# xacond00/mitsuba3-amvpt

Hardware: AMD Instinct MI355X
Metric: Msamples/sec (whole node), 8-view 1024² 64spp; per-pixel RMSE vs llvm_rgb (higher is better)
Workload: dtype f32; 1 GPU; M: cbox_grid.xml, 8-view 1024x1024 per view (quilt 4096x2048), 64 spp (4 passes x 16), G=8, sa_mis, adaptive 0, max_depth 8, rr_depth 5, seed 0; partition=equal lane counts, film_bytes_per_gpu=134217728

## Files before the change

include/amvpt.h:

```cpp
#ifndef AMVPT_H
#define AMVPT_H

#include <stddef.h>
#include <stdint.h>

#ifdef __cplusplus
extern "C" {
#endif

#define AMVPT_ABI_VERSION 10

typedef enum amvpt_status {
    AMVPT_OK = 0,
    AMVPT_ERR_INVALID = 1,
    AMVPT_ERR_HIP = 2,
    AMVPT_ERR_OOM = 3,
    AMVPT_ERR_UNSUPPORTED = 4,
    AMVPT_ERR_NO_DEVICE = 5
} amvpt_status;


enum {
    AMVPT_SHAPE_RECTANGLE = 0,
    AMVPT_SHAPE_MESH = 1,
    AMVPT_SHAPE_SPHERE = 2
};

typedef struct amvpt_shape_desc {
    uint32_t type;
    int32_t bsdf;
    int32_t emitter;
    uint32_t flip_normals;
    float to_world[16];
    float to_object[16];
    uint32_t vertex_count;
    uint32_t face_count;
    const float *positions;
    const float *normals;
    const float *texcoords;
    const uint32_t *faces;
    float center[3];
    float radius;
} amvpt_shape_desc;

enum {
    AMVPT_BSDF_DIFFUSE = 0,
    AMVPT_BSDF_ROUGHCONDUCTOR = 1,
    AMVPT_BSDF_TWOSIDED = 2
};
enum { AMVPT_MICROFACET_BECKMANN = 0, AMVPT_MICROFACET_GGX = 1 };

typedef struct amvpt_bsdf_desc {
    uint32_t type;
    int32_t nested[2];
    float reflectance[3];
    uint32_t distribution;
    uint32_t sample_visible;
    float alpha_u, alpha_v;
    float eta[3], k[3];
    uint32_t has_specular_reflectance;
    float specular_reflectance[3];
} amvpt_bsdf_desc;

// ... 121 lines not shown
amvpt_status amvpt_scene_destroy(amvpt_scene *scene);
amvpt_status amvpt_scene_stats(const amvpt_scene *scene, uint32_t *n_nodes, uint32_t *n_prims);
amvpt_status amvpt_scene_desc_boxes(const amvpt_scene_desc *d, uint32_t *n_boxes);

uint32_t amvpt_film_channels(const amvpt_params *params);

amvpt_status amvpt_render(amvpt_scene *scene, const amvpt_view_desc *views,
                          const amvpt_params *params, uint64_t lane_begin,
                          uint64_t lane_end, float *film_device, void *stream,
                          amvpt_counters *counters);

amvpt_status amvpt_render_records(amvpt_scene *scene, const amvpt_view_desc *views,
                                  const amvpt_params *params, uint32_t pass,
                                  uint64_t lane_begin, uint64_t lane_end, float *film_device,
                                  float *records_device, void *stream);

amvpt_status amvpt_plan(const amvpt_params *params, uint32_t *spp, uint32_t *spp_per_pass,
                        uint32_t *n_passes, uint64_t *lanes_per_pass);

amvpt_status amvpt_develop(const float *film_device, float *out_device, uint32_t width,
                           uint32_t height, uint32_t film_alpha, void *stream);

amvpt_status amvpt_set_chunk_lanes(uint64_t chunk_lanes);
amvpt_status amvpt_set_traversal(uint32_t mode);
amvpt_status amvpt_set_bvh_build(uint32_t max_leaf_prims, float traversal_cost);

typedef int (*amvpt_exchange_fn)(void *ctx, uint64_t local_count, uint64_t *prefix, uint64_t *total);
amvpt_status amvpt_set_adaptive_exchange(amvpt_exchange_fn fn, void *ctx);


typedef struct amvpt_lane_set {
    uint64_t lane_begin, lane_end;
    uint32_t rect_x0, rect_y0, rect_width, rect_height;
} amvpt_lane_set;

typedef struct amvpt_film_window {
    float *film;
    uint32_t x0, y0, width, height;
    uint32_t *overflow;
    uint64_t overflow_capacity;
} amvpt_film_window;

typedef int (*amvpt_run_exchange_fn)(void *ctx, uint32_t n_runs, const uint64_t *run_lane_begin,
                                     const uint64_t *run_count, uint64_t *run_prefix, uint64_t *total);

enum {
    AMVPT_OPT_GENERIC_KERNELS = 1u,
    AMVPT_OPT_WAVEFRONT_SUFFIX = 2u,
    AMVPT_OPT_SPLIT_NEE = 4u,
    AMVPT_OPT_ONE_STREAM = 8u,
    AMVPT_OPT_NO_BINNING = 32u,
    AMVPT_OPT_NO_BOX_SCREEN = 64u,
    AMVPT_OPT_THREADED_BVH = 128u,
    AMVPT_OPT_DETERMINISTIC = 16u
};
typedef struct amvpt_render_opts {
    uint64_t chunk_lanes;
    uint32_t traversal;
    uint32_t flags;
    amvpt_run_exchange_fn exchange;
    void *exchange_ctx;
    float *records;
    uint32_t record_pass;
    uint32_t budget_mib;
} amvpt_render_opts;

amvpt_status amvpt_render_ex(amvpt_scene *scene, const amvpt_view_desc *views, const amvpt_params *params,
                             const amvpt_lane_set *lanes, const amvpt_film_window *film, void *stream,
                             const amvpt_render_opts *opts, amvpt_counters *counters);

amvpt_status amvpt_film_accumulate(float *quilt, uint32_t quilt_width, uint32_t quilt_height, uint32_t channels,
                                   const float *window, uint32_t x0, uint32_t y0, uint32_t width, uint32_t height,
                                   const uint32_t *overflow_entries, uint64_t n_entries, void *stream);

amvpt_status amvpt_release_device_memory(int device);

amvpt_status amvpt_scene_bvh2(const amvpt_scene *scene, uint32_t *n_nodes2, uint32_t *depth);

#ifdef __cplusplus
}
#endif

#endif
```

mitsuba3-amvpt_amd/amvpt/__init__.py:

```python
import ctypes
import os

import numpy as np

_HERE = os.path.dirname(os.path.abspath(__file__))
LIB_DIR = os.environ.get("AMVPT_LIB_DIR") or os.path.join(os.path.dirname(_HERE), "lib")
HIP_LIB_PATH = os.path.join(LIB_DIR, "libamvpt_hip.so")
HOST_LIB_PATH = os.path.join(LIB_DIR, "libamvpt_host.so")

u32, i32, u64, f32, f64 = ctypes.c_uint32, ctypes.c_int32, ctypes.c_uint64, ctypes.c_float, ctypes.c_double


class ShapeDesc(ctypes.Structure):
    _fields_ = [("type", u32), ("bsdf", i32), ("emitter", i32), ("flip_normals", u32),
                ("to_world", f32 * 16), ("to_object", f32 * 16),
                ("vertex_count", u32), ("face_count", u32),
                ("positions", ctypes.POINTER(f32)), ("normals", ctypes.POINTER(f32)),
                ("texcoords", ctypes.POINTER(f32)), ("faces", ctypes.POINTER(u32)),
                ("center", f32 * 3), ("radius", f32)]


class BsdfDesc(ctypes.Structure):
    _fields_ = [("type", u32), ("nested", i32 * 2), ("reflectance", f32 * 3), ("distribution", u32),
                ("sample_visible", u32), ("alpha_u", f32), ("alpha_v", f32), ("eta", f32 * 3),
# ... 20 lines not shown


class Params(ctypes.Structure):
    _fields_ = [(n, u32) for n in (
        "integrator", "max_depth", "rr_depth", "hide_emitters", "sa_reuse", "sa_mis", "fast_mis",
        "debug", "adaptive", "spp_pass_lim", "reuse_count", "spp", "seed", "base_seed", "n_views",
        "multisensor", "grid_x", "grid_y", "reverse_x", "reverse_y", "film_width", "film_height",
        "film_alpha", "rfilter")] + [("rfilter_stddev", f32), ("batch", u32), ("crop_offset_x", u32),
                                      ("crop_offset_y", u32), ("full_width", u32), ("full_height", u32)]


class Counters(ctypes.Structure):
    _fields_ = [("lanes", u64), ("passes", u64), ("vertices", u64), ("reuse_lanes", u64),
                ("visibility_rays", u64), ("view_splats", u64), ("adaptive_lanes", u64),
                ("kernel_ms_primary", f64), ("kernel_ms_bounce", f64), ("kernel_ms_splat", f64),
                ("total_ms", f64), ("splat_fallback", u64),
                ("shadow_rays", u64), ("kernel_ms", f64 * 12), ("kernel_launches", u64 * 12),
                ("record_bytes", u64), ("nonfinite_samples", u64), ("negative_samples", u64),
                ("pushed_paths", u64), ("film_overflow", u64), ("film_range_drops", u64),
                ("chunk_lanes", u64), ("buffer_sets", u64), ("arena_bytes", u64),
                ("primary_record_bytes", u64), ("splat_record_bytes", u64)]

    def as_dict(self):
        d = {k: getattr(self, k) for k, _ in self._fields_}
        for k in ("kernel_ms", "kernel_launches"):
            d[k] = {name: d[k][i] for i, name in enumerate(KERNELS)}
        return d


class LaneSet(ctypes.Structure):
    _fields_ = [("lane_begin", u64), ("lane_end", u64), ("rect_x0", u32), ("rect_y0", u32),
                ("rect_width", u32), ("rect_height", u32)]


class FilmWindow(ctypes.Structure):
    _fields_ = [("film", ctypes.c_void_p), ("x0", u32), ("y0", u32), ("width", u32), ("height", u32),
                ("overflow", ctypes.c_void_p), ("overflow_capacity", u64)]


RunExchangeFn = ctypes.CFUNCTYPE(ctypes.c_int, ctypes.c_void_p, u32, ctypes.POINTER(u64), ctypes.POINTER(u64),
                                 ctypes.POINTER(u64), ctypes.POINTER(u64))


class RenderOpts(ctypes.Structure):
    _fields_ = [("chunk_lanes", u64), ("traversal", u32), ("flags", u32), ("exchange", RunExchangeFn),
                ("exchange_ctx", ctypes.c_void_p), ("records", ctypes.c_void_p), ("record_pass", u32),
                ("budget_mib", u32)]


OPT_GENERIC_KERNELS, OPT_WAVEFRONT_SUFFIX, OPT_SPLIT_NEE, OPT_ONE_STREAM, OPT_DETERMINISTIC = 1, 2, 4, 8, 16
OPT_NO_BINNING = 32
OPT_NO_BOX_SCREEN = 64
OPT_THREADED_BVH = 128


def wrap_run_exchange(fn):
    def cb(_ctx, n, begins, counts, prefix, total):
        try:
            pre, tot = fn([int(begins[i]) for i in range(n)], [int(counts[i]) for i in range(n)])
            for i in range(n):
                prefix[i] = int(pre[i])
            total[0] = int(tot)
            return 0
        except Exception:
            return 1
    return RunExchangeFn(cb)


KERNELS = ("k_prim_hit", "k_prim_req", "k_vis", "k_mv_primary", "k_raygen", "k_extend", "k_bounce", "k_shadow",
           "k_splat", "k_suffix", "k_select", "k_bin")


INTEGRATOR_MVPATH, INTEGRATOR_PATH = 0, 1
EMITTER_AREA, EMITTER_CONSTANT = 0, 1
_hip = None
_host = None


def hip_lib():
    global _hip
    if _hip is None:
        if not os.path.exists(HIP_LIB_PATH):
            raise RuntimeError("libamvpt_hip.so missing: run `make -C mitsuba3-amvpt_amd` "
                               "(__graft_entry__.build()); the product path has no fallback")
        L = ctypes.CDLL(HIP_LIB_PATH, mode=ctypes.RTLD_GLOBAL)
        L.amvpt_last_error.restype = ctypes.c_char_p
        L.amvpt_abi_version.restype = u32
        L.amvpt_film_channels.restype = u32
        for fn in ("amvpt_device_count", "amvpt_set_device", "amvpt_scene_create", "amvpt_scene_destroy",
                   "amvpt_scene_stats", "amvpt_render", "amvpt_render_records", "amvpt_plan",
                   "amvpt_develop", "amvpt_set_chunk_lanes", "amvpt_set_traversal",
                   "amvpt_set_adaptive_exchange", "amvpt_set_bvh_build", "amvpt_render_ex", "amvpt_scene_desc_boxes",
                   "amvpt_release_device_memory"):
            if hasattr(L, fn):
                getattr(L, fn).restype = ctypes.c_int
        L.amvpt_render.argtypes = [ctypes.c_void_p, ctypes.c_void_p, ctypes.POINTER(Params), u64, u64,
                                   ctypes.c_void_p, ctypes.c_void_p, ctypes.POINTER(Counters)]
        if hasattr(L, "amvpt_render_ex"):
            L.amvpt_render_ex.argtypes = [ctypes.c_void_p, ctypes.c_void_p, ctypes.POINTER(Params),
                                          ctypes.POINTER(LaneSet), ctypes.POINTER(FilmWindow), ctypes.c_void_p,
                                          ctypes.POINTER(RenderOpts), ctypes.POINTER(Counters)]
        L.amvpt_render_records.argtypes = [ctypes.c_void_p, ctypes.c_void_p, ctypes.POINTER(Params), u32, u64,
                                           u64, ctypes.c_void_p, ctypes.c_void_p, ctypes.c_void_p]
        L.amvpt_scene_create.argtypes = [ctypes.POINTER(SceneDesc), ctypes.POINTER(ctypes.c_void_p)]
        L.amvpt_scene_destroy.argtypes = [ctypes.c_void_p]
        L.amvpt_scene_stats.argtypes = [ctypes.c_void_p, ctypes.POINTER(u32), ctypes.POINTER(u32)]
# ... 326 lines not shown
```

mitsuba3-amvpt_amd/csrc/amvpt_render.hip:

```cpp
#include <hip/hip_runtime.h>
#include <rocprofiler-sdk-roctx/roctx.h>

#include <algorithm>
#include <chrono>
#include <cmath>
#include <cstdlib>
#include <cstring>
#include <map>
#include <memory>
#include <mutex>
#include <type_traits>

#include "internal.h"
#include "dbsdf.h"

#if defined(AMVPT_SHADOW_TU) || defined(AMVPT_GROUP_TU)
#define AMVPT_TU_LOCAL static
#else
#define AMVPT_TU_LOCAL
#endif

namespace amvpt {

#if !defined(AMVPT_SHADOW_TU) && !defined(AMVPT_GROUP_TU)
// ... 18 lines not shown
        Hit best{kInf, 0.f, 0.f, -1};
        uint32_t best_orig = 0xffffffffu;
        outer_closest(sc, r, best, best_orig);
        return trace_closest2<walk_sph<kWalk>()>(sc, r, best, best_orig);
    }
    return trace_closest<kWalk == WALK_UNI, AMVPT_WALK_WW, walk_sph<kWalk>()>(sc, r);
}
template <int kWalk> AD bool walk_any(const SceneRef &sc, const Ray &r) {
    if (kWalk == WALK_BRUTE || kWalk == WALK_BRUTE_NS) return brute_any<kWalk == WALK_BRUTE>(sc, r);
    if (kWalk != WALK_UNI && sc.stk) return trace_any2<walk_sph<kWalk>()>(sc, r, outer_any(sc, r, false));
    return trace_any<kWalk == WALK_UNI, AMVPT_WALK_WW, walk_sph<kWalk>()>(sc, r);
}

struct KParams {
    uint32_t W, H, C;
    uint32_t bvh2, stk_off_ext, stk_off_any;
    uint32_t spp_pp, log_spp, pow2;
    uint32_t max_depth, rr_depth;
    uint32_t sa_mis, fast_mis, debug, n_adapt;
    uint32_t G;
    uint32_t multisensor, batch, n_views, gx, gy, rev_x, rev_y, sres_x, sres_y;
    uint32_t needs_ap;
    uint32_t box, coalesce_single, path_box_pos, is_mvpath;
    uint32_t seed_value;
    uint32_t trav_mode;
    uint32_t sph;
    uint32_t win_rs;
    uint32_t adapt_seed;
    uint32_t pass_seed;
    uint64_t range_begin;
    uint32_t rect, rect_x0, rect_y0, run_len;
    uint32_t fx0, fy0, fw, fh;
    uint32_t *overflow;
    uint64_t ov_cap;
    float inv_w, inv_h;
    uint32_t off_x, off_y;
    float adj_ox, adj_oy, nc_ox, nc_oy;
    float adapt_w;
    FilterCoeffs filt;
    uint64_t chunk_begin;
    uint32_t chunk_n;
    uint32_t record;
    uint32_t row_splat;
    uint32_t tile_w;
    double rcp_tpr, rcp_run_len, rcp_n_adapt;
    uint32_t adapt_pass;
    uint32_t valid_ray0;
    uint32_t vs_stride;
    unsigned long long *film_fx;
    float *film_base;
    unsigned long long *fx_drops;
    unsigned long long *rng_in, *rng_out;
    uint32_t box_screen;
    float bin_lo[3], bin_scale[3];
};

AD Pcg pass_rng(const KParams &P, uint32_t lane, uint64_t v) {
    uint32_t v0, v1;
    tea4(P.seed_value, lane, v0, v1);
    Pcg rng;
    if (P.rng_in) {
        rng.state = P.rng_in[v];
        rng.inc = (((uint64_t) v1) << 1) | 1u;
    } else {
        rng.seed(v0, v1);
    }
    return rng;
}

constexpr int kQPlanes = 5;
struct Bufs {
    float4 *q_in[kQPlanes];
    float4 *q_out[kQPlanes];
    uint32_t *cnt_in, *cnt_out;
    uint32_t qcap;
    float4 *lane_out;
    float4 *lrec[4];
    float4 *vrec;
    float *film;
    float *records;
    unsigned long long *stats;
    uint8_t *amask;
    const uint32_t *asel;
    const uint32_t *run_delta;
    float4 *hit;
    float4 *nee[2];
    float2 *nee_gb;
    uint32_t *cnt_nee;
    float4 *vreq[3];
    unsigned long long *occ;
    uint4 *vreq_w[8];
    uint4 *lmask_w[24];
    float *vstate;
    float4 *sray[2];
    float2 *sgb;
    uint16_t *key_out, *key_in, *key_nee;
};


constexpr int kPrimBlock = 128;
enum { F_PDF, F_JP, F_PDFM, F_WX, F_WY, F_WZ, VS_FIELDS };
constexpr int kVsFieldsDiff = 2;

__host__ __device__ inline bool scene_uniform(uint32_t n_nodes, uint32_t mode) {
    return mode == 1u || (mode == 0u && n_nodes <= kUniformNodeLimit);
}
// ... 2213 lines not shown

#ifndef AMVPT_BOUNCE_TAB
#define AMVPT_BOUNCE_TAB 1
#endif
#ifndef AMVPT_PRIM_TAB
#define AMVPT_PRIM_TAB 1
#endif
#ifndef AMVPT_PRIM_SLOT_ORDER
#define AMVPT_PRIM_SLOT_ORDER 1
#endif
#ifndef AMVPT_DEFER_SAMPLE
#define AMVPT_DEFER_SAMPLE 1
#endif
#ifndef AMVPT_PAIR_REGS
#define AMVPT_PAIR_REGS 1
#endif
#ifndef AMVPT_PDF_REGS
#define AMVPT_PDF_REGS 1
#endif
#ifndef AMVPT_DIFF_REGS
#define AMVPT_DIFF_REGS 0
#endif
template <int G, bool kDiff> __host__ __device__ constexpr bool diff_regs() {
    return AMVPT_DIFF_REGS && AMVPT_PAIR_REGS && kDiff && G >= 2 && G <= 8;
}
template <int G, bool kDiff> __host__ __device__ constexpr bool pdf_in_regs() {
    return (AMVPT_PAIR_REGS && AMVPT_PDF_REGS && !kDiff && G >= 2 && G <= 8) || diff_regs<G, kDiff>();
}
template <int G, bool kDiff> __host__ __device__ constexpr int vs_fields() {
    return kDiff ? (diff_regs<G, kDiff>() ? 0 : kVsFieldsDiff) : VS_FIELDS - (pdf_in_regs<G, kDiff>() ? 1 : 0);
}
#ifndef AMVPT_FUSED_TWO_STREAMS
#define AMVPT_FUSED_TWO_STREAMS 0
#endif
#ifndef AMVPT_CHUNK_STREAMS
#define AMVPT_CHUNK_STREAMS 4
#endif
#ifndef AMVPT_TILE_SLOTS
#define AMVPT_TILE_SLOTS 1
#endif
#ifndef AMVPT_PDF_ROW
#define AMVPT_PDF_ROW 1
#endif
#ifndef AMVPT_COH_UNI
#define AMVPT_COH_UNI 1
#endif
#ifndef AMVPT_WAVE_DIFF
#define AMVPT_WAVE_DIFF 1
#endif
#ifndef AMVPT_PRIM_WAVES
#define AMVPT_PRIM_WAVES 1
#endif
template <int G> constexpr int prim_block() { return G > 0 ? kPrimBlock : 64; }
template <int G, bool kTab, bool kDiff, bool kGenRec>
AD void mv_primary_lane(const KParams &P, const DScene &S, const SceneRef &sc, const DView *V, const Bufs &B,
                        float *const vs, const uint32_t vs_stride, const uint32_t slot, const uint32_t i, const bool ok) {
    const int Gn = group_size<G>(P);
    constexpr bool kPdfRegs = pdf_in_regs<G, kDiff>();
    constexpr bool kJpRegs = diff_regs<G, kDiff>();
#define VSF(f, k) vs[(((f) - (kPdfRegs ? 1 : 0)) * Gn + (k)) * vs_stride]
    PathState ps;
    bool push = false;
    unsigned long long st_reuse = 0, st_vis = 0;
    if (ok) {
        const float4 hitv = B.hit[i];
        VMask<G> occm = 0;
#pragma unroll
        for (int k = 0; k < Gn; ++k) mset(occm, k, occluded_n(B, (uint32_t) Gn, i, k));
        const uint32_t n = P.chunk_n;
        const PrimRay pr = primary_raygen(P, V, i);
        Pcg rng = pr.rng;
        const uint32_t v1 = pr.v1, p_idx = pr.p_idx;
        const float apx = pr.apx, apy = pr.apy;
        const Ray pray = pr.ray;
        float *const vw = kGenRec ? vrec_compact(B, Gn, n) : reinterpret_cast<float *>(B.vrec);
        float4 *const vR = B.vrec, *const vB = B.vrec + (size_t) Gn * n;
        auto view_of = [&](int k) -> uint32_t { return group_view_n((uint32_t) Gn, p_idx, k); };
        auto put_view = [&](int k, float w, C3 res, C3 bv, uint32_t vf) {
            const size_t o = (size_t) k * n + slot;
            if (kDiff) {
                vw[o] = w;
            } else {
                vR[o] = make_float4(res.r, res.g, res.b, w);
                vB[o] = make_float4(bv.r, bv.g, bv.b, bitsf(vf));
            }
        };
        VMask<G> vmask = 0, imask = 0;
        float w0 = 1.f;
        C3 R0 = c3(0.f);
        C3 Dp = c3(0.f);
        C3 Bv = c3(0.f);
        f3 hp = mk(0.f, 0.f, 0.f);
        bool records_done = false, reuse_l = false, direct_l = false;
        uint32_t nf_bits = 0;
        VMask<G> smask = 0;

        bool valid_ray = P.valid_ray0 != 0 && P.max_depth != 0, adapt_mask = false;
        float pdfW = 1.f;
        bool should_mis = P.sa_mis != 0;
        if (P.max_depth != 0) {
            SI si = compute_si(sc, pray, hit_of(hitv));
            bool p_hit = si.valid();
            hp = si.p;
            int32_t em = si_emitter(sc, si);
            bool direct_em = em >= 0;
            C3 emitted = c3(0.f);
            if (direct_em) emitted = emitter_eval(sc, em, si, true);
            int32_t b = p_hit ? S.shapes[si.shape].bsdf : -1;
            bool bsdf_smooth = (bsdf_flags(S.bsdfs, b) & BF_Smooth) != 0;
            bool active_em = p_hit && bsdf_smooth;
            float e1 = rng.next_1d(), e2 = rng.next_1d();
            DSamp ds;
            C3 em_w;
            if (sample_emitter_direction(sc, si, e1, e2, active_em, ds, em_w) && mget(occm, 0))
                occlude_emitter_sample(ds, em_w);
            active_em = active_em && ds.pdf != 0.f;
            direct_l = active_em;
            f3 wo = si.sh.to_local(ds.d);
            float rand_1 = rng.next_1d();
            float r2a = rng.next_1d(), r2b = rng.next_1d();
            (void) rand_1;
            C3 bsdf_val;
            float direct_pdf;
            bsdf_eval_pdf<kDiff>(S.bsdfs, b, CTX_ALL, si.wi, wo, true, bsdf_val, direct_pdf);
            BSample bsmp;
            C3 bsdf_weight;
            bsdf_sample<kDiff>(S.bsdfs, b, CTX_ALL, si.wi, r2a, r2b, true, bsmp, bsdf_weight);
            bool flag_delta = (bsmp.type & BF_Delta) != 0, flag_null = (bsmp.type & BF_Null) != 0;
            bool flag_diff = (bsmp.type & BF_Diffuse) != 0;
            bool delta = flag_delta || flag_null, p_not_delta = !delta && p_hit;
            bool reuse = !direct_em && p_not_delta && bsdf_smooth;
            reuse_l = reuse;
            st_reuse += reuse ? 1 : 0;
            bool p_face = si.wi.z > 0.f;
            if (should_mis) {
                BD bd;
                bd.bsdf = b;
                bd.alpha = bsdf_roughness<kDiff>(S.bsdfs, b, si.wi);
                bd.sqr_a = fmsub(bd.alpha, bd.alpha, 1.f);
                bd.rsqrt_a = rsqrt_(bd.alpha);
                bd.diffuse = flag_diff;
                bd.reuse = reuse;
                Surf p0 = camera_sample_surface(V[view_of(0)], si, p_hit, apx, apy);
                const float pdf0 = p0.pdf, Jp0 = p0.Jp, iJp0 = p_hit ? rcp(p0.Jp) : 0.f;
                if (!kPdfRegs) VSF(F_PDF, 0) = pdf0;
                float rJp[kJpRegs ? G : 1];
                if constexpr (kJpRegs) {
                    rJp[0] = Jp0;
#pragma unroll
                    for (int j = 1; j < G; ++j) rJp[j] = 0.f;
                } else {
                    VSF(F_JP, 0) = Jp0;
                }
                mset(vmask, 0, p_hit);
                mset(imask, 0, p_hit);
                const f3 wo_r0 = reflect_l(si.wi);
                VMask<G> wpos = p_face ? 1u : 0u;
                if (!kDiff) {
                    VSF(F_WX, 0) = si.wi.x; VSF(F_WY, 0) = si.wi.y; VSF(F_WZ, 0) = si.wi.z;
                    VSF(F_PDFM, 0) = bd.diffuse ? 1.f : (P.fast_mis ? sqr(normalize(si.wi + wo_r0).z)
                                                                   : bsdf_pdf(S.bsdfs, b, CTX_GLOSSY, si.wi, wo_r0, p_hit));
                }
                auto wi_of = [&](int k) -> f3 {
                    if (kDiff) return k == 0 ? si.wi : mk(0.f, 0.f, mget(wpos, k) ? 1.f : -1.f);
                    return mk(VSF(F_WX, k), VSF(F_WY, k), VSF(F_WZ, k));
                };
                auto mat_pdf = [&](f3 wik, float pdfM, bool active) -> float {
                    if (bd.diffuse) return 1.f;
                    return P.fast_mis ? tv_pdf_fast(wo_r0, wik, pdfM, bd, active)
                                      : tv_pdf(S.bsdfs, wo_r0, wik, pdfM, bd, active);
                };
                float rPdf[kPdfRegs ? G : 1];
                if constexpr (kPdfRegs) {
#pragma unroll
                    for (int j = 0; j < G; ++j) rPdf[j] = 0.f;
                }
                float n_direct = 1.f, n_indir = 2.f;
                int rep_k = 0;
                (void) rep_k;
#pragma unroll 1
                for (int k = 1; k < Gn; ++k) {
                    Surf r = camera_sample_surface(V[view_of(k)], si, bd.reuse, apx, apy);
                    bool valid = r.valid && (r.face == p_face) && r.Jp > 0.f;
                    if (valid) {
                        ++st_vis;
                        valid = !mget(occm, k);
                    }
                    f3 wik = si.sh.to_local(r.d);
                    float pdf_Mat = 1.f;
                    if (!kDiff) {
                        VSF(F_WX, k) = wik.x; VSF(F_WY, k) = wik.y; VSF(F_WZ, k) = wik.z;
                        f3 wor = reflect_l(wik);
                        float pdfM = P.fast_mis ? sqr(normalize(wik + wor).z)
                                                : bsdf_pdf(S.bsdfs, b, CTX_GLOSSY, wik, wor, valid);
                        VSF(F_PDFM, k) = pdfM;
                        pdf_Mat = mat_pdf(wik, pdfM, valid);
                    } else {
                        mset(wpos, k, wik.z > 0.f);
                    }
                    float J = r.Jp * iJp0;
                    float pdf_J = J > 1.f ? rcp(J) : J;
                    float pdf_Sel = pdf_Mat * pdf_J;
                    valid = valid && (rng.next_1d() < pdf_Sel);
                    if constexpr (kJpRegs) {
#pragma unroll
                        for (int j = 1; j < G; ++j) rJp[j] = j == k ? r.Jp : rJp[j];
                    } else {
                        VSF(F_JP, k) = r.Jp;
                    }
                    if constexpr (kPdfRegs) {
                        const float pk = valid ? r.pdf : 0.f;
#pragma unroll
                        for (int j = 1; j < G; ++j) rPdf[j] = j == k ? pk : rPdf[j];
                    } else {
                        VSF(F_PDF, k) = valid ? r.pdf : 0.f;
                    }
                    bool indirect = valid, direct = valid;
                    bool replace = n_indir * rng.next_1d() < 1.f;
                    C3 bvk;
                    float bpk;
                    BSample bsk;
                    C3 bwk;
                    bsdf_eval_pdf<kDiff>(S.bsdfs, b, CTX_ALL, wik, wo, valid, bvk, bpk);
                    direct = direct && bpk > 0.f;
                    direct_pdf += direct ? bpk : 0.f;
                    n_direct += (float) direct;
                    if (!kDiff) {
#if AMVPT_DEFER_SAMPLE
                        indirect = indirect && bsdf_sample_type(S.bsdfs, b, CTX_ALL, wik, valid) == bsmp.type;
                        if (indirect && replace) rep_k = k;
#else
                        bsdf_sample(S.bsdfs, b, CTX_ALL, wik, r2a, r2b, valid, bsk, bwk);
                        indirect = indirect && bsk.type == bsmp.type;
                        if (indirect && replace) bsmp.wo = bsk.wo;
#endif
                    }
                    (void) replace;
                    n_indir += (float) indirect;
                    mset(vmask, k, valid);
// ... 122 lines not shown
                            if (j == k) continue;
                            float pdf_J = vmin(sqr(VSF(F_JP, j) * iJpk), 1.f);
                            acc = fmadd(VSF(F_PDF, j), pdf_J, acc);
                        }
                        acc = cond ? acc : 0.f;
                    }
                    pdfSum += acc;
                    const float wk = pdf_lk / pdfSum;
                    bool valid = mget(imask, k);
                    C3 res = c3(0.f), bv = c3(0.f);
                    float bp;
                    if (kDiff) {
                        bp = (valid && mget(wpos, k)) ? bp_d : 0.f;
                    } else {
                        res = csel(k == 0, emitted, c3(0.f));
                        if (active_em && vk) {
                            C3 bvk = bsdf_val;
                            if (k > 0) {
                                float bpk;
                                bsdf_eval_pdf<kDiff>(S.bsdfs, b, CTX_ALL, wik, wo, true, bvk, bpk);
                            }
                            res = cfma(bvk, emis_mis, res);
                        }
                        if (k == 0) R0 = res;
                        bsdf_eval_pdf<kDiff>(S.bsdfs, b, CTX_ALL, wik, bsmp.wo, valid, bv, bp);
                        if (k == 0) {
                            bv = csel(p_not_delta, bv, bsdf_weight);
                            bp = p_not_delta ? bp : bsmp.pdf;
                            valid = valid && (bp > 0.f || delta);
                        }
                    }
                    bool pvalid = bp > 0.f;
                    valid = valid && ((k == 0 && !kDiff) ? (pvalid || delta) : pvalid);
                    bp = valid ? bp : 0.f;
                    bv = csel(valid, bv, c3(0.f));
                    pdf += bp;
                    n_ind += (float) valid;
                    if (!valid) mclr(imask, k);
                    if (k == 0) w0 = wk;
                    else put_view(k, wk, res, bv, (vk ? VF_VALID : 0u) | (valid ? VF_INDIRECT : 0u));
                    if (k == 0 && !kDiff) Bv = bv;
                }
                bsmp.pdf = p_not_delta ? pdf / n_ind : bsmp.pdf;
                adapt_mask = p_hit && !flag_null && (n_ind <= 1.f);
                records_done = true;
            } else {
                mset(vmask, 0, p_hit);
#pragma unroll 1
                for (int k = 1; k < Gn; ++k) {
                    Surf r = camera_sample_surface(V[view_of(k)], si, reuse, apx, apy);
                    bool valid = r.valid && (r.face == p_face) && r.Jp > 0.f;
                    if (valid) {
                        ++st_vis;
                        valid = !mget(occm, k);
                    }
                    mset(vmask, k, valid);
                }
                float mis_em = ds.delta ? 1.f : mis_weight(ds.pdf, direct_pdf);
                R0 = emitted;
                if (active_em) R0 = cfma(bsdf_val, em_w * mis_em, R0);
            }
            Ray pd_ray = spawn_ray(si.p, si.n, si.sh.to_world(bsmp.wo));
            C3 thr = csel(should_mis, c3(1.f), bsdf_weight);
            valid_ray = valid_ray || (p_hit && !flag_null);
            bool pd_active = p_hit;
            if (!should_mis) pd_active = pd_active && (cmax(thr) != 0.f);
            if (P.max_depth <= 1) pd_active = false;
            pdfW = p_not_delta ? rcp(bsmp.pdf) : 1.f;
            if (pd_active) {
                ps.ray = pd_ray;
                ps.thr = thr;
                ps.res = c3(0.f);
                ps.eta_zero = bsmp.eta == 0.f;
                ps.prev_pdf = bsmp.pdf;
                ps.depth = p_hit ? 1u : 0u;
                ps.prev_delta = flag_delta;
                ps.valid_ray = false;
                ps.prev_p = si.p;
                ps.idx = slot;
                ps.rng_state = rng.state;
                ps.rng_seq = v1;
                push = true;
            }
            if (!p_hit) w0 = 1.f;
            mset(vmask, 0, true);
        }
        if (!push) B.lane_out[slot] = make_float4(0.f, 0.f, 0.f, 0.f);
        if (P.max_depth == 0) {
            vmask = 0u;
            imask = 0u;
            w0 = 0.f;
        }
        const uint32_t lflags = (valid_ray ? LF_VALIDRAY : 0u) | (adapt_mask ? LF_ADAPT : 0u) |
                                (should_mis ? LF_MIS : 0u) | (reuse_l ? LF_REUSE : 0u) | (direct_l ? LF_DIRECT : 0u) |
                                (nf_bits << 8) | mlow16(smask) | (kGenRec ? LF_DIFFW : 0u);
        B.lrec[0][slot] = make_float4(R0.r, R0.g, R0.b, pdfW);
        B.lrec[1][slot] = make_float4(Dp.r, Dp.g, Dp.b, bitsf(lflags));
        B.lrec[2][slot] = make_float4(Bv.r, Bv.g, Bv.b, bitsf(mlow16(vmask) >> 16 | mlow16(imask)));
        if constexpr (G <= 0) {
            constexpr int NP = mask_planes<G>();
            mstore(B.lmask_w, slot, vmask);
            mstore(B.lmask_w + NP, slot, imask);
            mstore(B.lmask_w + 2 * NP, slot, smask);
        }
        B.lrec[3][slot] = make_float4(hp.x, hp.y, hp.z, 0.f);
        put_view(0, w0, R0, Bv, (mget(vmask, 0) ? VF_VALID : 0u) | (mget(imask, 0) ? VF_INDIRECT : 0u));
        if (!records_done) {
#pragma unroll 1
            for (int k = 1; k < Gn; ++k)
                put_view(k, P.max_depth != 0 ? 1.f : 0.f, c3(0.f), c3(0.f), (mget(vmask, k)) ? VF_VALID : 0u);
        }
    }
    const uint32_t qslot = push_slot(push, B.cnt_out, B.qcap);
    if (push) store_state(B.q_out, qslot, ps);
    if (B.stats) {
        stat_add(B.stats, 1, st_reuse);
        stat_add(B.stats, 2, st_vis);
        stat_add(B.stats, 0, (ok && P.max_depth != 0) ? 1ull : 0ull);
        stat_add(B.stats, 8, push ? 1ull : 0ull);
        stat_add(B.stats, 10, ok ? (unsigned long long) ((kDiff ? 4 : 32) * Gn) : 0ull);
    }
}
#undef VSF

AD bool wave_diffuse(const KParams &P, const DScene &S, const SceneRef &sc, const Bufs &B, uint32_t i, bool ok) {
    bool dl = true;
    if (ok && P.max_depth != 0) {
        const int32_t prim = (int32_t) fbits(B.hit[i].w);
        if (prim >= 0) {
            const int32_t b = S.shapes[sc.prims[prim].shape].bsdf;
            dl = b < 0 || S.bsdfs[b].type == BSDF_DIFFUSE;
        }
    }
    return !wave_any(!dl);
}
template <int G, bool kTab, bool kDiff, bool kDW = false>
__global__ void __launch_bounds__(prim_block<G>(), AMVPT_PRIM_WAVES) k_mv_primary(KParams P, const DScene *Sp, const DView *V, Bufs B) {
    constexpr int kPB = prim_block<G>();
    extern __shared__ __attribute__((aligned(16))) char lds[];
    DScene S = *Sp;
    const uint32_t vs_off = kTab ? S.tab_bytes + views_lds_bytes(P.n_views) : 0u;
    SceneRef sc = stage_scene<kTab, false>(S, lds, P.trav_mode, &V, P.n_views);
    const bool vs_glob = G <= 0 && B.vstate != nullptr;
    const uint32_t vs_stride = vs_glob ? P.vs_stride : (uint32_t) kPB;
    float *const vs = vs_glob ? B.vstate + (blockIdx.x * blockDim.x + threadIdx.x)
                              : reinterpret_cast<float *>(lds + vs_off) + threadIdx.x;
#if AMVPT_PRIM_SLOT_ORDER
    const uint32_t slot = blockIdx.x * blockDim.x + threadIdx.x;
    bool ok = slot < P.chunk_n;
    const uint32_t i = ok ? slot_lane(P, slot) : 0u;
#else
    const uint32_t i = blockIdx.x * blockDim.x + threadIdx.x;
    bool ok = i < P.chunk_n;
    const uint32_t slot = ok ? lane_slot(P, i) : 0u;
#endif
    if constexpr (kDiff) {
        mv_primary_lane<G, kTab, true, false>(P, S, sc, V, B, vs, vs_stride, slot, i, ok);
    } else if (kDW) {
        if (wave_diffuse(P, S, sc, B, i, ok)) mv_primary_lane<G, kTab, true, true>(P, S, sc, V, B, vs, vs_stride, slot, i, ok);
    } else {
        if (!(AMVPT_WAVE_DIFF && wave_diffuse(P, S, sc, B, i, ok)))
            mv_primary_lane<G, kTab, false, false>(P, S, sc, V, B, vs, vs_stride, slot, i, ok);
    }
}



#ifndef AMVPT_SPLAT_SKIP
#define AMVPT_SPLAT_SKIP 1
#endif
#ifndef AMVPT_SPLAT_BVW
#define AMVPT_SPLAT_BVW 1
#endif
#ifndef AMVPT_SPLAT_WAVES
#define AMVPT_SPLAT_WAVES 5
#endif
template <int G, int C, bool kDiff, bool kRow, bool kWin = true, bool kRec = true>
__global__ void __launch_bounds__(kSplatBlock, AMVPT_SPLAT_WAVES) k_splat_multi(KParams P, const DView *V, Bufs B) {
    const bool rec_ = kRec && P.record != 0, dbg_ = kRec && P.debug != 0;
    __shared__ typename std::conditional<kRow, WaveLds<C>, SplatLds<C>>::type L;
    if (kRow) wave_lds_init(reinterpret_cast<WaveLds<C> &>(L));
    else splat_lds_init(reinterpret_cast<SplatLds<C> &>(L));
    auto put = [&](float x, float y, const float *vals, bool valid, bool coalesce, int buf, uint32_t *fb) {
        if constexpr (kRow) {
            wave_put<C, kWin>(P, B.film, L, x, y, vals, valid, coalesce, fb);
        } else {
            if (P.film_fx) direct_put<C, kWin>(P, B.film, x, y, vals, valid, coalesce);
            else block_put<C>(P, B.film, L, buf, x, y, vals, valid, coalesce, fb);
        }
    };
    const uint32_t slot = blockIdx.x * kSplatBlock + threadIdx.x;
    const bool ok = slot < P.chunk_n;
    const uint32_t i = ok ? slot_lane(P, slot) : 0u;
    const uint32_t n = P.chunk_n;
    float4 l0 = make_float4(0.f, 0.f, 0.f, 0.f), l1 = l0, l2 = l0, l3 = l0, lo = l0;
    if (ok) { l0 = B.lrec[0][slot]; l1 = B.lrec[1][slot]; l2 = B.lrec[2][slot]; l3 = B.lrec[3][slot]; lo = B.lane_out[slot]; }
    const int Gn = group_size<G>(P);
    const uint32_t lflags = fbits(l1.w);
    VMask<G> vmask = 0u, imask = 0u, smask = 0u;
    if constexpr (G <= 0) {
        constexpr int NP = mask_planes<G>(), NW = mask_words<G>();
        if (ok) { vmask = mload<NW>(B.lmask_w, slot); imask = mload<NW>(B.lmask_w + NP, slot); smask = mload<NW>(B.lmask_w + 2 * NP, slot); }
    } else {
        vmask = fbits(l2.w) & 0xffffu; imask = fbits(l2.w) >> 16; smask = lflags >> 16;
    }
    const float qnan = __builtin_nanf("");
    const float pdfW = l0.w;
    const C3 R0 = C3{l0.x, l0.y, l0.z}, Dp = C3{l1.x, l1.y, l1.z}, Bv = C3{l2.x, l2.y, l2.z};
    const f3 hp = mk(l3.x, l3.y, l3.z);
    if (ok && B.amask) B.amask[P.chunk_begin + i] = (lflags & LF_ADAPT) ? 1u : 0u;
// ... 87 lines not shown
        if (dbg_) {
            if (k > 0) break;
            pack_vals(P, c3(adapt_mask ? 1.f : 0.f), alpha, 1.f, vals);
            put(x, y, vals, ok, true, 0, nullptr);
            continue;
        }
        pack_vals(P, v, alpha, weight, vals);
        check_sample(P, vals, valid, nonfinite, negative);
        put(x, y, vals, valid, k == 0, k & 1, &fallback);
        splats += valid ? 1 : 0;
        if (ok && rec_) {
            float *rr = B.records + ((size_t) i * Gn + k) * 8;
            rr[0] = x; rr[1] = y; rr[2] = v.r; rr[3] = v.g; rr[4] = v.b; rr[5] = alpha; rr[6] = weight;
            rr[7] = valid ? 1.f : 0.f;
        }
    }
    if (B.stats) {
        stat_add(B.stats, 3, splats); stat_add(B.stats, 4, fallback);
        stat_add(B.stats, 6, nonfinite); stat_add(B.stats, 7, negative);
        const uint32_t vb = !ok ? 0u : kd ? 4u * views_read
                                          : 16u * ((rec_ ? views_read : mpopc(vmask)) + (mis ? mpopc(imask) : 0u));
        stat_add(B.stats, 11, vb);
    }
}

AMVPT_TU_LOCAL __global__ void k_develop(const float *film, float *out, uint32_t npx, uint32_t alpha) {
    uint32_t p = blockIdx.x * blockDim.x + threadIdx.x;
    if (p >= npx) return;
    uint32_t C = alpha ? 5u : 4u, T = alpha ? 4u : 3u;
    const float *src = film + (size_t) p * C;
    float w = src[C - 1];
    float d = w == 0.f ? 1.f : w;
    for (uint32_t c = 0; c < T; ++c) out[(size_t) p * T + c] = src[c] / d;
}

void launch_shadow(int walk, bool bin, dim3 grid, size_t lds, hipStream_t st, const KParams &P, const DScene *dS, const Bufs &B)
#ifdef AMVPT_SHADOW_TU
{
    if (bin && walk == WALK_LANE_TRI) hipLaunchKernelGGL(HIP_KERNEL_NAME(k_shadow<WALK_LANE_TRI, true>), grid, dim3(256), lds, st, P, dS, B);
    else if (bin && walk == WALK_LANE_NS) hipLaunchKernelGGL(HIP_KERNEL_NAME(k_shadow<WALK_LANE_NS, true>), grid, dim3(256), lds, st, P, dS, B);
    else if (bin && walk == WALK_LANE) hipLaunchKernelGGL(HIP_KERNEL_NAME(k_shadow<WALK_LANE, true>), grid, dim3(256), lds, st, P, dS, B);
    else if (walk == WALK_BRUTE_NS) hipLaunchKernelGGL(HIP_KERNEL_NAME(k_shadow<WALK_BRUTE_NS>), grid, dim3(256), lds, st, P, dS, B);
    else if (walk == WALK_BRUTE) hipLaunchKernelGGL(HIP_KERNEL_NAME(k_shadow<WALK_BRUTE>), grid, dim3(256), lds, st, P, dS, B);
    else if (walk == WALK_UNI) hipLaunchKernelGGL(HIP_KERNEL_NAME(k_shadow<WALK_UNI>), grid, dim3(256), lds, st, P, dS, B);
    else if (walk == WALK_LANE_TRI) hipLaunchKernelGGL(HIP_KERNEL_NAME(k_shadow<WALK_LANE_TRI>), grid, dim3(256), lds, st, P, dS, B);
    else if (walk == WALK_LANE_NS) hipLaunchKernelGGL(HIP_KERNEL_NAME(k_shadow<WALK_LANE_NS>), grid, dim3(256), lds, st, P, dS, B);
    else hipLaunchKernelGGL(HIP_KERNEL_NAME(k_shadow<WALK_LANE>), grid, dim3(256), lds, st, P, dS, B);
}
#else
;
#endif

struct AbKnobs {
    bool fuse_prim = true, row_splat = true, brute = true, fuse_nee = true, fuse_suffix = true;
    uint32_t win_rs = AMVPT_WIN_RS, fused_blocks = AMVPT_FUSED_BLOCKS;
};
inline const AbKnobs &ab_knobs() {
    static const AbKnobs k = [] {
        AbKnobs r;
#ifdef AMVPT_AB_KNOBS
        auto off = [](const char *n) { const char *e = std::getenv(n); return e && e[0] == '0'; };
        r.fuse_prim = !off("AMVPT_FUSE_PRIM");
        r.row_splat = !off("AMVPT_ROW_SPLAT");
        r.brute = !off("AMVPT_BRUTE");
        r.fuse_nee = !off("AMVPT_FUSE_NEE");
        r.fuse_suffix = !off("AMVPT_FUSE_SUFFIX");
        if (const char *e = std::getenv("AMVPT_WIN_RS")) r.win_rs = (uint32_t) std::strtoul(e, nullptr, 0) % 32u;
        if (const char *e = std::getenv("AMVPT_FUSED_BLOCKS"))
            r.fused_blocks = std::max<uint32_t>(1, std::min<uint32_t>(64, (uint32_t) std::strtoul(e, nullptr, 0)));
#endif
        return r;
    }();
    return k;
}

#ifndef AMVPT_FLUSH_MARKS
#define AMVPT_FLUSH_MARKS 1
#endif
struct KTimer {
    static constexpr size_t kPairs = 128;
    bool on = false;
    hipError_t err = hipSuccess;
    hipEvent_t ev[2 * kPairs] = {};
    int kid[kPairs] = {};
    size_t n = 0;
    double ms[AMVPT_K_COUNT] = {};
    uint64_t launches[AMVPT_K_COUNT] = {};
    void init(bool enable) {
        on = enable;
        if (!on) return;
        for (auto &e : ev)
            if (err == hipSuccess) err = hipEventCreate(&e);
    }
    void flush() {
        if (!on || n == 0 || err != hipSuccess) return;
        for (size_t i = 0; i < n && err == hipSuccess; ++i) {
            err = hipEventSynchronize(ev[2 * i + 1]);
            if (err != hipSuccess) break;
            float t = 0.f;
            err = hipEventElapsedTime(&t, ev[2 * i], ev[2 * i + 1]);
            ms[kid[i]] += t;
            launches[kid[i]] += 1;
        }
        n = 0;
    }
    void begin(int k, hipStream_t st) {
        if (!on || err != hipSuccess) return;
        if (n == kPairs) flush();
        kid[n] = k;
        err = hipEventRecord(ev[2 * n], st);
    }
    void end(hipStream_t st) {
        if (!on || err != hipSuccess) return;
        err = hipEventRecord(ev[2 * n + 1], st);
        ++n;
    }
    hipEvent_t mark_ev = nullptr;
    void mark(hipStream_t st) {
        if (on || !AMVPT_FLUSH_MARKS) return;
        if (!mark_ev && hipEventCreate(&mark_ev) != hipSuccess) return;
        (void) hipEventRecord(mark_ev, st);
    }
    ~KTimer() {
        for (auto &e : ev)
            if (e) (void) hipEventDestroy(e);
        if (mark_ev) (void) hipEventDestroy(mark_ev);
    }
};

void launch_prim_hit(bool uni, dim3 grid, size_t lds_bvh, hipStream_t st, const KParams &P, const DScene *S,
                     const DView *V, const Bufs &B)
#if !defined(AMVPT_SHADOW_TU) && !defined(AMVPT_GROUP_TU)
{
    if (uni) hipLaunchKernelGGL(HIP_KERNEL_NAME(k_prim_hit<true>), grid, dim3(256), lds_bvh, st, P, S, V, B);
    else hipLaunchKernelGGL(HIP_KERNEL_NAME(k_prim_hit<false>), grid, dim3(256), lds_bvh, st, P, S, V, B);
}
#else
;
#endif
#ifdef AMVPT_GROUP_TU
template <int G> inline int group_size_host(const KParams &P) { return G > 0 ? G : (int) P.G; }
template <int G>
void launch_primary(uint32_t cn, size_t lds_tab, size_t lds_bvh, hipStream_t st, const KParams &P,
                           const DScene *S, const DView *V, const Bufs &B, bool tab, bool uni, bool diff, KTimer &T) {
    constexpr int kPB = prim_block<G>(), kVW = vis_waves<G>();
    const dim3 g256((cn + 255) / 256), g64((cn + 63) / 64), gp((cn + kPB - 1) / kPB);
    const size_t lds_view = B.vstate ? 0u : (size_t) (diff ? vs_fields<G, true>() : vs_fields<G, false>()) * group_size_host<G>(P) * kPB * sizeof(float);
    if (uni && ab_knobs().fuse_prim) {
        T.begin(AMVPT_K_PRIM_HIT, st);
        if (tab && diff && P.sph == 0) hipLaunchKernelGGL(HIP_KERNEL_NAME(k_prim_hit_req<G, true, true, 0>), g256, dim3(256), lds_tab, st, P, S, V, B);
        else if (tab && P.sph == 0) hipLaunchKernelGGL(HIP_KERNEL_NAME(k_prim_hit_req<G, true, false, 0>), g256, dim3(256), lds_tab, st, P, S, V, B);
        else if (tab && diff && P.sph == 2) hipLaunchKernelGGL(HIP_KERNEL_NAME(k_prim_hit_req<G, true, true, 2>), g256, dim3(256), lds_tab, st, P, S, V, B);
        else if (tab && P.sph == 2) hipLaunchKernelGGL(HIP_KERNEL_NAME(k_prim_hit_req<G, true, false, 2>), g256, dim3(256), lds_tab, st, P, S, V, B);
        else if (tab && diff) hipLaunchKernelGGL(HIP_KERNEL_NAME(k_prim_hit_req<G, true, true>), g256, dim3(256), lds_tab, st, P, S, V, B);
        else if (tab) hipLaunchKernelGGL(HIP_KERNEL_NAME(k_prim_hit_req<G, true, false>), g256, dim3(256), lds_tab, st, P, S, V, B);
        else if (diff) hipLaunchKernelGGL(HIP_KERNEL_NAME(k_prim_hit_req<G, false, true>), g256, dim3(256), lds_tab, st, P, S, V, B);
        else hipLaunchKernelGGL(HIP_KERNEL_NAME(k_prim_hit_req<G, false, false>), g256, dim3(256), lds_tab, st, P, S, V, B);
        T.end(st);
    } else {
        T.begin(AMVPT_K_PRIM_HIT, st);
        launch_prim_hit(uni, g256, lds_bvh, st, P, S, V, B);
        T.end(st);
        T.begin(AMVPT_K_PRIM_REQ, st);
        if (tab && diff) hipLaunchKernelGGL(HIP_KERNEL_NAME(k_prim_req<G, true, true>), g256, dim3(256), lds_tab, st, P, S, V, B);
        else if (tab) hipLaunchKernelGGL(HIP_KERNEL_NAME(k_prim_req<G, true, false>), g256, dim3(256), lds_tab, st, P, S, V, B);
        else if (diff) hipLaunchKernelGGL(HIP_KERNEL_NAME(k_prim_req<G, false, true>), g256, dim3(256), lds_tab, st, P, S, V, B);
        else hipLaunchKernelGGL(HIP_KERNEL_NAME(k_prim_req<G, false, false>), g256, dim3(256), lds_tab, st, P, S, V, B);
        T.end(st);
    }
    T.begin(AMVPT_K_VIS, st);
    constexpr bool kVisPairs = vis_pairs<G, true>();
    const dim3 gvis = kVisPairs ? dim3((cn + 64 * AMVPT_VIS_RAYS - 1) / (64 * AMVPT_VIS_RAYS)) : g64;
    if (uni && P.sph == 0) hipLaunchKernelGGL(HIP_KERNEL_NAME(k_vis<G, true, 0>), gvis, dim3(64 * kVW), lds_bvh, st, P, S, V, B);
    else if (uni && P.sph == 2) hipLaunchKernelGGL(HIP_KERNEL_NAME(k_vis<G, true, 2>), gvis, dim3(64 * kVW), lds_bvh, st, P, S, V, B);
    else if (uni) hipLaunchKernelGGL(HIP_KERNEL_NAME(k_vis<G, true>), gvis, dim3(64 * kVW), lds_bvh, st, P, S, V, B);
    else hipLaunchKernelGGL(HIP_KERNEL_NAME(k_vis<G, false>), g64, dim3(64 * kVW), lds_bvh, st, P, S, V, B);
    T.end(st);
    T.begin(AMVPT_K_MV_PRIMARY, st);
    if (tab && diff) hipLaunchKernelGGL(HIP_KERNEL_NAME(k_mv_primary<G, true, true>), gp, dim3(kPB), lds_tab + lds_view, st, P, S, V, B);
    else if (diff) hipLaunchKernelGGL(HIP_KERNEL_NAME(k_mv_primary<G, false, true>), gp, dim3(kPB), lds_tab + lds_view, st, P, S, V, B);
    else {
        if (AMVPT_WAVE_DIFF) {
            const size_t lds_dw = B.vstate ? 0u : (size_t) vs_fields<G, true>() * group_size_host<G>(P) * kPB * sizeof(float);
            if (tab) hipLaunchKernelGGL(HIP_KERNEL_NAME(k_mv_primary<G, true, false, true>), gp, dim3(kPB), lds_tab + lds_dw, st, P, S, V, B);
            else hipLaunchKernelGGL(HIP_KERNEL_NAME(k_mv_primary<G, false, false, true>), gp, dim3(kPB), lds_tab + lds_dw, st, P, S, V, B);
        }
        if (tab) hipLaunchKernelGGL(HIP_KERNEL_NAME(k_mv_primary<G, true, false>), gp, dim3(kPB), lds_tab + lds_view, st, P, S, V, B);
        else hipLaunchKernelGGL(HIP_KERNEL_NAME(k_mv_primary<G, false, false>), gp, dim3(kPB), lds_tab + lds_view, st, P, S, V, B);
    }
    T.end(st);
}
template <int G>
void launch_splat(dim3 grid, hipStream_t st, const KParams &P, const DView *V, const Bufs &B, bool diff) {
    const bool row = AMVPT_WAVE_WIN && P.row_splat && P.C == 4 && !P.film_fx;
    const bool whole = P.fx0 == 0u && P.fy0 == 0u && P.fw == P.W && P.fh == P.H;
    if (P.C == 5 && diff) hipLaunchKernelGGL(HIP_KERNEL_NAME(k_splat_multi<G, 5, true, false>), grid, dim3(kSplatBlock), 0, st, P, V, B);
    else if (P.C == 5) hipLaunchKernelGGL(HIP_KERNEL_NAME(k_splat_multi<G, 5, false, false>), grid, dim3(kSplatBlock), 0, st, P, V, B);
    else if (diff && row && whole && !P.record && !P.debug) hipLaunchKernelGGL(HIP_KERNEL_NAME(k_splat_multi<G, 4, true, true, false, false>), grid, dim3(kSplatBlock), 0, st, P, V, B);
    else if (row && whole && !P.record && !P.debug) hipLaunchKernelGGL(HIP_KERNEL_NAME(k_splat_multi<G, 4, false, true, false, false>), grid, dim3(kSplatBlock), 0, st, P, V, B);
    else if (diff && row && whole) hipLaunchKernelGGL(HIP_KERNEL_NAME(k_splat_multi<G, 4, true, true, false>), grid, dim3(kSplatBlock), 0, st, P, V, B);
// ... 359 lines not shown
    const bool partial = rect || lane_begin != 0 || lane_end != L;
    const amvpt_run_exchange_fn exchange = opts.exchange;
    void *const exchange_ctx = opts.exchange_ctx;
    if (do_fill && partial && !exchange) {
        set_error("amvpt_render: adaptive > 0 over a lane range needs amvpt_set_adaptive_exchange "
                  "(or the whole frame: lane_begin = 0, lane_end = all lanes)");
        return AMVPT_ERR_UNSUPPORTED;
    }
    if (span == 0) {
        if (do_fill && partial)
            for (uint32_t pass = 0; pass < n_passes; ++pass) {
                uint64_t total = 0;
                if (exchange(exchange_ctx, 0, nullptr, nullptr, nullptr, &total) != 0) {
                    set_error("amvpt_render: adaptive count exchange failed");
                    return AMVPT_ERR_INVALID;
                }
            }
        if (counters) *counters = amvpt_counters{};
        return AMVPT_OK;
    }

    KParams P{};
    P.W = Pp.film_width; P.H = Pp.film_height; P.C = Pp.film_alpha ? 5 : 4;
    P.spp_pp = spp_pp;
    uint32_t log_spp = 0;
    while ((1u << log_spp) < spp_pp) ++log_spp;
    P.log_spp = log_spp;
    P.pow2 = (1u << log_spp) == spp_pp;
    P.max_depth = Pp.max_depth; P.rr_depth = Pp.rr_depth;
    P.sa_mis = Pp.sa_mis; P.fast_mis = Pp.fast_mis; P.debug = Pp.debug; P.n_adapt = n_adapt;
    P.G = G;
    P.multisensor = Pp.multisensor; P.batch = Pp.batch; P.n_views = Pp.n_views;
    P.needs_ap = 0;
    for (uint32_t v = 0; v < (Pp.multisensor && Pp.batch ? Pp.n_views : 1u); ++v)
        P.needs_ap |= views[v].type == AMVPT_CAMERA_THINLENS ? 1u : 0u;
    P.gx = Pp.grid_x ? Pp.grid_x : 1; P.gy = Pp.grid_y ? Pp.grid_y : 1;
    P.rev_x = Pp.reverse_x; P.rev_y = Pp.reverse_y;
    const uint32_t fullW = Pp.full_width ? Pp.full_width : P.W, fullH = Pp.full_height ? Pp.full_height : P.H;
    P.sres_x = fullW / P.gx; P.sres_y = fullH / P.gy;
    P.box = Pp.rfilter == AMVPT_RFILTER_BOX;
    P.coalesce_single = spp_pp >= 4;
    P.path_box_pos = (!is_mv && P.box) ? 1 : 0;
    P.is_mvpath = is_mv;
    P.inv_w = 1.f / (float) P.W;
    P.inv_h = 1.f / (float) P.H;
    P.off_x = Pp.crop_offset_x; P.off_y = Pp.crop_offset_y;
    P.adj_ox = -(float) P.off_x * P.inv_w;
    P.adj_oy = -(float) P.off_y * P.inv_h;
    P.nc_ox = (float) (-(int) P.off_x) - .5f;
    P.nc_oy = (float) (-(int) P.off_y) - .5f;
    P.adapt_w = 1.f / (float) (n_adapt + 1);
    P.trav_mode = trav;
    P.box_screen = (opts.flags & AMVPT_OPT_NO_BOX_SCREEN) ? 0u : 1u;
    for (int a = 0; a < 3; ++a) {
        const float ext = scene->root_hi[a] - scene->root_lo[a];
        P.bin_lo[a] = scene->root_lo[a];
        P.bin_scale[a] = ext > 0.f ? (float) (1u << kBinCellBits) / ext : 0.f;
    }
    P.sph = !scene->has_spheres ? 0u : (AMVPT_SPHERE_DEFER && scene->n_sph <= 64u) ? 2u : 1u;
    P.win_rs = K.win_rs;
    P.range_begin = rect ? 0 : lane_begin;
    P.rect = rect ? 1u : 0u;
    P.rect_x0 = rx0; P.rect_y0 = ry0;
    P.run_len = rect ? rw * spp_pp : 0u;
    P.fx0 = fwin.x0; P.fy0 = fwin.y0; P.fw = fwin.width; P.fh = fwin.height;
    P.overflow = whole_film ? nullptr : fwin.overflow;
    P.ov_cap = whole_film ? 0 : fwin.overflow_capacity;
    uint64_t overflow_before = 0, overflow_added = 0;
    if (P.overflow) {
        HIPCHK(hipMemcpyAsync(&overflow_before, P.overflow, 8, hipMemcpyDeviceToHost, st));
        HIPCHK(hipStreamSynchronize(st));
    }
    P.valid_ray0 = (!Pp.hide_emitters && scene->dev.environment >= 0) ? 1u : 0u;
    if (!P.box) gaussian_coeffs(Pp.rfilter_stddev, P.filt);
    {
        FilterCoeffs d;
        gaussian_coeffs(0.5f, d);
        const bool def_filt = !P.box && std::memcmp(&d, &P.filt, sizeof(d)) == 0 &&
                              std::memcmp(&d.c[0], &kDefaultFilterHost[0], sizeof(d.c)) == 0;
        P.row_splat = (K.row_splat && P.C == 4 && def_filt && P.pow2 && spp_pp >= 16) ? 1u : 0u;
    }
    {
        const uint64_t band = 4ull * QW * 16ull;
        P.tile_w = (AMVPT_TILE_SLOTS && P.row_splat && spp_pp == 16 && QW % 4 == 0 && !rect && lane_begin % band == 0 &&
                    span % band == 0 && span <= 0xffffffffull) ? QW : 0u;
    }

    std::vector<DView> hv(Pp.n_views);
    for (uint32_t v = 0; v < Pp.n_views; ++v) {
        const amvpt_view_desc &d = views[v];
        DView &o = hv[v];
        std::memcpy(o.to_world, d.to_world, 12 * sizeof(float));
        std::memcpy(o.to_world_inv, d.to_world_inv, 12 * sizeof(float));
        std::memcpy(o.sample_to_camera, d.sample_to_camera, 16 * sizeof(float));
        std::memcpy(o.camera_to_sample, d.camera_to_sample, 16 * sizeof(float));
        o.near_clip = d.near_clip; o.far_clip = d.far_clip; o.normalization = d.normalization; o.pad0 = 0.f;
        o.res[0] = d.resolution[0]; o.res[1] = d.resolution[1];
        o.pp[0] = d.pp_offset[0]; o.pp[1] = d.pp_offset[1];
        o.type = d.type;
        o.aperture_radius = d.aperture_radius;
        o.focus_distance = d.focus_distance;
        o.pad1 = 0.f;
    }

    const bool wide = G > kMaxG;
    const int mplanes = G > kMaxGWide ? mask_planes<-1>() : mask_planes<0>();
// ... 588 lines not shown
```

Baseline: 2113 Msamples/s.

## Fuse primary hit, visibility and vertex kernels into one MV-primary launch

For uniform all-diffuse scenes with compile-time group size and no spheres, the primary closest-hit trace and the per-view occlusion tests are moved into the MV-primary kernel. Their results no longer pass through the hit and occlusion buffers between separate launches. This removes kernel launches and global-memory round trips, and occlusion rays are traced lazily only for views whose reprojection is valid. The cost is higher register pressure and possible divergence in the fused kernel, addressed by a waves-per-EU launch bound. A new option flag restores the split path.

```diff
diff --git a/include/amvpt.h b/include/amvpt.h
--- a/include/amvpt.h
+++ b/include/amvpt.h
@@ -8,7 +8,7 @@
 extern "C" {
 #endif
 
-#define AMVPT_ABI_VERSION 10
+#define AMVPT_ABI_VERSION 11
 
 typedef enum amvpt_status {
     AMVPT_OK = 0,
@@ -236,6 +236,7 @@
     AMVPT_OPT_NO_BINNING = 32u,
     AMVPT_OPT_NO_BOX_SCREEN = 64u,
     AMVPT_OPT_THREADED_BVH = 128u,
+    AMVPT_OPT_SPLIT_PRIMARY = 256u,
     AMVPT_OPT_DETERMINISTIC = 16u
 };
 typedef struct amvpt_render_opts {
diff --git a/mitsuba3-amvpt_amd/amvpt/__init__.py b/mitsuba3-amvpt_amd/amvpt/__init__.py
--- a/mitsuba3-amvpt_amd/amvpt/__init__.py
+++ b/mitsuba3-amvpt_amd/amvpt/__init__.py
@@ -96,6 +96,7 @@
 OPT_NO_BINNING = 32
 OPT_NO_BOX_SCREEN = 64
 OPT_THREADED_BVH = 128
+OPT_SPLIT_PRIMARY = 256
 
 
 def wrap_run_exchange(fn):
diff --git a/mitsuba3-amvpt_amd/csrc/amvpt_render.hip b/mitsuba3-amvpt_amd/csrc/amvpt_render.hip
--- a/mitsuba3-amvpt_amd/csrc/amvpt_render.hip
+++ b/mitsuba3-amvpt_amd/csrc/amvpt_render.hip
@@ -94,6 +94,7 @@
     unsigned long long *fx_drops;
     unsigned long long *rng_in, *rng_out;
     uint32_t box_screen;
+    uint32_t split_prim;
     float bin_lo[3], bin_scale[3];
 };
 
@@ -2413,9 +2414,10 @@
 #define AMVPT_PRIM_WAVES 1
 #endif
 template <int G> constexpr int prim_block() { return G > 0 ? kPrimBlock : 64; }
-template <int G, bool kTab, bool kDiff, bool kGenRec>
+template <int G, bool kTab, bool kDiff, bool kGenRec, bool kFuse = false>
 AD void mv_primary_lane(const KParams &P, const DScene &S, const SceneRef &sc, const DView *V, const Bufs &B,
                         float *const vs, const uint32_t vs_stride, const uint32_t slot, const uint32_t i, const bool ok) {
+    static_assert(!kFuse || (kDiff && !kGenRec && G >= 2), "the fused primary vertex: all-diffuse compile-time groups");
     const int Gn = group_size<G>(P);
     constexpr bool kPdfRegs = pdf_in_regs<G, kDiff>();
     constexpr bool kJpRegs = diff_regs<G, kDiff>();
@@ -2424,10 +2426,13 @@
     bool push = false;
     unsigned long long st_reuse = 0, st_vis = 0;
     if (ok) {
-        const float4 hitv = B.hit[i];
+        float4 hitv = make_float4(0.f, 0.f, 0.f, 0.f);
         VMask<G> occm = 0;
-#pragma unroll
-        for (int k = 0; k < Gn; ++k) mset(occm, k, occluded_n(B, (uint32_t) Gn, i, k));
+        if constexpr (!kFuse) {
+            hitv = B.hit[i];
+#pragma unroll
+            for (int k = 0; k < Gn; ++k) mset(occm, k, occluded_n(B, (uint32_t) Gn, i, k));
+        }
         const uint32_t n = P.chunk_n;
         const PrimRay pr = primary_raygen(P, V, i);
         Pcg rng = pr.rng;
@@ -2460,7 +2465,18 @@
         float pdfW = 1.f;
         bool should_mis = P.sa_mis != 0;
         if (P.max_depth != 0) {
-            SI si = compute_si(sc, pray, hit_of(hitv));
+            Hit phit;
+            if constexpr (kFuse) phit = trace_closest<true, 0, 0>(sc, pray);
+            else phit = hit_of(hitv);
+            SI si = compute_si(sc, pray, phit);
+            auto occluded = [&](int k, f3 to) -> bool {
+                if constexpr (kFuse) {
+                    if (k > 0) to = camera_point(V[view_of(k)], apx, apy);
+                    return trace_any<true, 0, 0>(sc, spawn_ray_to(si.p, si.n, to));
+                } else {
+                    return mget(occm, k);
+                }
+            };
             bool p_hit = si.valid();
             hp = si.p;
             int32_t em = si_emitter(sc, si);
@@ -2473,7 +2489,7 @@
             float e1 = rng.next_1d(), e2 = rng.next_1d();
             DSamp ds;
             C3 em_w;
-            if (sample_emitter_direction(sc, si, e1, e2, active_em, ds, em_w) && mget(occm, 0))
+            if (sample_emitter_direction(sc, si, e1, e2, active_em, ds, em_w) && occluded(0, ds.p))
                 occlude_emitter_sample(ds, em_w);
             active_em = active_em && ds.pdf != 0.f;
             direct_l = active_em;
@@ -2545,7 +2561,7 @@
                     bool valid = r.valid && (r.face == p_face) && r.Jp > 0.f;
                     if (valid) {
                         ++st_vis;
-                        valid = !mget(occm, k);
+                        valid = !occluded(k, hp);
                     }
                     f3 wik = si.sh.to_local(r.d);
                     float pdf_Mat = 1.f;
@@ -2774,7 +2790,7 @@
                     bool valid = r.valid && (r.face == p_face) && r.Jp > 0.f;
                     if (valid) {
                         ++st_vis;
-                        valid = !mget(occm, k);
+                        valid = !occluded(k, hp);
                     }
                     mset(vmask, k, valid);
                 }
@@ -2856,8 +2872,11 @@
     }
     return !wave_any(!dl);
 }
-template <int G, bool kTab, bool kDiff, bool kDW = false>
-__global__ void __launch_bounds__(prim_block<G>(), AMVPT_PRIM_WAVES) k_mv_primary(KParams P, const DScene *Sp, const DView *V, Bufs B) {
+#ifndef AMVPT_PRIM_FUSE_WAVES
+#define AMVPT_PRIM_FUSE_WAVES 6
+#endif
+template <int G, bool kTab, bool kDiff, bool kDW = false, bool kFuse = false>
+__global__ void __launch_bounds__(prim_block<G>(), kFuse ? AMVPT_PRIM_FUSE_WAVES : AMVPT_PRIM_WAVES) k_mv_primary(KParams P, const DScene *Sp, const DView *V, Bufs B) {
     constexpr int kPB = prim_block<G>();
     extern __shared__ __attribute__((aligned(16))) char lds[];
     DScene S = *Sp;
@@ -2877,7 +2896,7 @@
     const uint32_t slot = ok ? lane_slot(P, i) : 0u;
 #endif
     if constexpr (kDiff) {
-        mv_primary_lane<G, kTab, true, false>(P, S, sc, V, B, vs, vs_stride, slot, i, ok);
+        mv_primary_lane<G, kTab, true, false, kFuse>(P, S, sc, V, B, vs, vs_stride, slot, i, ok);
     } else if (kDW) {
         if (wave_diffuse(P, S, sc, B, i, ok)) mv_primary_lane<G, kTab, true, true>(P, S, sc, V, B, vs, vs_stride, slot, i, ok);
     } else {
@@ -3071,7 +3090,7 @@
 #endif
 
 struct AbKnobs {
-    bool fuse_prim = true, row_splat = true, brute = true, fuse_nee = true, fuse_suffix = true;
+    bool fuse_prim = true, fuse_vertex = true, row_splat = true, brute = true, fuse_nee = true, fuse_suffix = true;
     uint32_t win_rs = AMVPT_WIN_RS, fused_blocks = AMVPT_FUSED_BLOCKS;
 };
 inline const AbKnobs &ab_knobs() {
@@ -3080,6 +3099,7 @@
 #ifdef AMVPT_AB_KNOBS
         auto off = [](const char *n) { const char *e = std::getenv(n); return e && e[0] == '0'; };
         r.fuse_prim = !off("AMVPT_FUSE_PRIM");
+        r.fuse_vertex = !off("AMVPT_FUSE_VERTEX");
         r.row_splat = !off("AMVPT_ROW_SPLAT");
         r.brute = !off("AMVPT_BRUTE");
         r.fuse_nee = !off("AMVPT_FUSE_NEE");
@@ -3165,6 +3185,14 @@
     constexpr int kPB = prim_block<G>(), kVW = vis_waves<G>();
     const dim3 g256((cn + 255) / 256), g64((cn + 63) / 64), gp((cn + kPB - 1) / kPB);
     const size_t lds_view = B.vstate ? 0u : (size_t) (diff ? vs_fields<G, true>() : vs_fields<G, false>()) * group_size_host<G>(P) * kPB * sizeof(float);
+    if constexpr (G >= 2) {
+        if (uni && ab_knobs().fuse_prim && ab_knobs().fuse_vertex && !P.split_prim && tab && diff && P.sph == 0) {
+            T.begin(AMVPT_K_MV_PRIMARY, st);
+            hipLaunchKernelGGL(HIP_KERNEL_NAME(k_mv_primary<G, true, true, false, true>), gp, dim3(kPB), lds_tab + lds_view, st, P, S, V, B);
+            T.end(st);
+            return;
+        }
+    }
     if (uni && ab_knobs().fuse_prim) {
         T.begin(AMVPT_K_PRIM_HIT, st);
         if (tab && diff && P.sph == 0) hipLaunchKernelGGL(HIP_KERNEL_NAME(k_prim_hit_req<G, true, true, 0>), g256, dim3(256), lds_tab, st, P, S, V, B);
@@ -3630,6 +3658,7 @@
     P.adapt_w = 1.f / (float) (n_adapt + 1);
     P.trav_mode = trav;
     P.box_screen = (opts.flags & AMVPT_OPT_NO_BOX_SCREEN) ? 0u : 1u;
+    P.split_prim = (opts.flags & AMVPT_OPT_SPLIT_PRIMARY) ? 1u : 0u;
     for (int a = 0; a < 3; ++a) {
         const float ext = scene->root_hi[a] - scene->root_lo[a];
         P.bin_lo[a] = scene->root_lo[a];
```

Result: faster. 2350 Msamples/s (median of 6 runs) (+11.2%).
